# Lagrange-Labs/mapreduce-plonky2

Measured on AMD Instinct MI355X. Metric: leaf proofs/sec (whole node) + NTT GB/s vs HBM peak, 2^20-row table build, 1/2/4/8 GPU, higher is better.
Workload: dtype u64 (Goldilocks field)

## Files before the change

### __graft_entry__.py

```python
import importlib
import os
import subprocess
import sys

ROOT = os.path.dirname(os.path.abspath(__file__))
PKG = os.path.join(ROOT, "mapreduce-plonky2_amd")


def build():
    env = dict(os.environ)
    subprocess.check_call(["make", "-s", "-j8", "-C", os.path.join(PKG, "csrc")], env=env)
    subprocess.check_call(["make", "-s", "-C", os.path.join(ROOT, "oracle")], env=env)
    subprocess.check_call(["make", "-s", "-C", os.path.join(ROOT, "tests", "devfield")], env=env)
    subprocess.check_call(["make", "-s", "-C", os.path.join(ROOT, "tests", "devfield_mulc")], env=env)
    subprocess.check_call(["make", "-s", "-C", os.path.join(ROOT, "tests", "devfield_mulk")], env=env)
    sys.path.insert(0, ROOT)
    mod = importlib.import_module("mapreduce-plonky2_amd")
    assert os.path.exists(mod.LIB_PATH)
    mod.load()


def smoke():
    import numpy as np
    sys.path.insert(0, ROOT)
    sys.path.insert(0, os.path.join(ROOT, "tests"))
    mp2 = importlib.import_module("mapreduce-plonky2_amd")
    import oracle as O
    ctx = mp2.Context(0)
    log_n, w = 10, 12
    vals = O.rand_field((w, 1 << log_n), 0xC0FFEE01)
    b = mp2.PolynomialBatch.from_values(ctx, vals, 3, 4)
    coeffs = O.fft(vals, inverse=True)
    cap = O.merkle_cap(O.merkle_build(O.lde_leaves(coeffs, 3), 4), 4)
    assert np.array_equal(b.coeffs, coeffs), "iNTT mismatch vs oracle"
    assert np.array_equal(b.cap, cap), "Merkle cap mismatch vs oracle"
    b.free()
    import ctypes
    import circuits as C
    ckt = C.build(5, C.ALL_KINDS, 1)
    ofp = O.standard_params(5, (ckt.num_constants + C.NUM_ROUTED, C.NUM_WIRES, 20, 16), pow_bits=6, num_queries=4)
    fp = mp2.FriParams()
    ctypes.memmove(ctypes.byref(fp), ctypes.byref(ofp), ctypes.sizeof(fp))
    cd = O.rand_field(4, 2)
    pr = mp2.BatchedProver(ctx, fp, 1)
    pr.set_preprocessed(ctx.to_device(ckt.pre))
    pr.enable_permutation(C.NUM_ROUTED, 8)
    pr.enable_quotient()
    pr.set_gates(ckt.gates, ckt.num_selectors)
    pr.prove([ctx.to_device(ckt.wires[None]), None, None], ctx.to_device(cd), ctx.to_device(ckt.pi_hash[None]))
    caps, openings, proofs = pr.results()
    oc, oo, op, bgao = C.prove(ckt, ofp, cd)
    assert np.array_equal(caps[0], oc) and np.array_equal(openings[0], oo) and np.array_equal(proofs[0], op), "proof mismatch vs oracle"
    assert O.pcs_verify(ofp, cd, ckt.pi_hash, caps[0], openings[0], proofs[0]) == 0, "FRI verifier rejects"
    assert C.identity_check(ckt, ofp, openings[0], bgao) == 0, "PLONK identity fails"
    ver = mp2.Verifier(ctx, fp, caps[0][0], cd, ckt.gates, ckt.num_selectors, capacity=2)
    words = np.concatenate([ckt.pi_hash, caps[0][1:].ravel(), openings[0].ravel(), proofs[0]])
    bad = words.copy()
    bad[4 + 3 * fp.cap_words + 9] ^= np.uint64(1)
    st = ver.verify(np.stack([words, bad])).tolist()
    assert st[0] == 0 and st[1] != 0, f"device verifier: {st}"
    ver.free()
    pr.free()
    R = importlib.import_module("mapreduce-plonky2_amd.recursion")
    FW = importlib.import_module("mapreduce-plonky2_amd.framework")
    data = O.rand_field(4, 0xC0FFEE03)
    mc = R.map_circuit(data)
    prog = mp2.WitnessProgram(mc)
    wires, pi_hash, pis = prog.run(data[None])
    assert np.array_equal(wires[0], mc.wires), "witness program != builder"
    n = 1 << mc.log_n
    d_in, d_w, d_pr = ctx.to_device(data[None]), ctx.alloc(135 * n * 8), ctx.alloc(prog.probe.size * 8)
    prog.run_dev(ctx, d_in, 1, d_w, d_pr)
    assert np.array_equal(d_w.download((135, n)), mc.wires), "device witness replay != builder"
    assert np.array_equal(d_pr.download((prog.probe.size,))[:4], pi_hash[0])
    cp = FW.CircuitProver(ctx, mc, 1, witness_check=True, pow_bits=8, num_queries=6)
    cp.prove(ctx.to_device(wires), ctx.to_device(pi_hash))
    assert cp.pr.witness_status().tolist() == [0]
    c2, o2, p2 = cp.results()
    mfp = C.oracle_params(mc, pow_bits=8, num_queries=6)
    assert C.verify(mc, mfp, cp.circuit_digest, pi_hash[0], c2[0], o2[0], p2[0]) == 0, "oracle verifier rejects the map proof"
    assert int(pis[0][0]) == sum(int(x) for x in data if int(x) % 2 == 0) % O.P
    cp.free()
    ctx.close()
    print("smoke ok: commit_from_values(12 x 2^10) == oracle; prove(2^5 rows, 24 gates) == oracle and verifies (oracle and device verifier); "
          "map circuit (real, witness program on host and device) proves and verifies")


if __name__ == "__main__":
    build()
    if len(sys.argv) > 1 and sys.argv[1] == "smoke":
        smoke()
```

### mapreduce-plonky2_amd/csrc/fri.hip

```cpp
#include "fri.h"
#include "poseidon_wave.cuh"

namespace mp2g {

template <int V>
__device__ void ch_duplex(ChState& c) {
  for (u32 i = 0; i < c.n_in; i++) c.state[i] = c.in[i];
  c.n_in = 0;
  u64 s[12];
#pragma unroll
  for (int i = 0; i < 12; i++) s[i] = c.state[i];
  perm<V>(s);
#pragma unroll
  for (int i = 0; i < 12; i++) c.state[i] = s[i];
#pragma unroll
  for (int i = 0; i < 8; i++) c.out[i] = s[i];
  c.n_out = 8;
}
template <int V>
__global__ void ch_kernel(ChState* st, u32 B, const u64* obs, u64 obs_bstride, u32 n_obs, u64* out, u64 out_bstride, u32 n_get) {
  u32 b = blockIdx.x * blockDim.x + threadIdx.x;
  if (b >= B) return;
  ChState c = st[b];
  const u64* o = obs + b * obs_bstride;
  for (u32 i = 0; i < n_obs; i++) {
    c.n_out = 0;
    c.in[c.n_in++] = o[i];
    if (c.n_in == 8) ch_duplex<V>(c);
  }
  u64* dst = out + b * out_bstride;
  for (u32 i = 0; i < n_get; i++) {
    if (c.n_in || !c.n_out) ch_duplex<V>(c);
    dst[i] = c.out[--c.n_out];
  }
  st[b] = c;
}
__global__ void __launch_bounds__(64) ch_wave_kernel(ChState* st, u32 B, const u64* obs, u64 obs_bstride, u32 n_obs, u64* out,
                                                     u64 out_bstride, u32 n_get) {
  const u32 gid = blockIdx.x * blockDim.x + threadIdx.x;
  const u32 braw = gid >> 4, l = gid & 15;
  const bool active = braw < B;
  const u32 b = active ? braw : B - 1;
  ChState* c = st + b;
  u64 x = l < 12 ? c->state[l] : 0;
  u64 inb = l < 8 ? c->in[l] : 0, outb = l < 8 ? c->out[l] : 0;
  u32 n_in = c->n_in, n_out = c->n_out;
  const u64* o = obs + b * obs_bstride;
  auto duplex = [&]() {
    if (l < n_in) x = inb;
    n_in = 0;
    x = wp2_perm(x, (int)l);
    outb = x;
    n_out = 8;
  };
  for (u32 i = 0; i < n_obs; i++) {
    u64 e = o[i];
    n_out = 0;
    if (l == n_in) inb = e;
    if (++n_in == 8) duplex();
  }
  u64* dst = out + b * out_bstride;
  for (u32 i = 0; i < n_get; i++) {
    if (n_in || !n_out) duplex();
    --n_out;
    if (active && l == n_out) dst[i] = outb;
  }
  if (!active) return;
  if (l < 12) c->state[l] = x;
  if (l < 8) { c->in[l] = inb; c->out[l] = outb; }
  if (l == 0) { c->n_in = n_in; c->n_out = n_out; }
}
__global__ void ch_init_kernel(ChState* st, u32 B) {
  u32 b = blockIdx.x * blockDim.x + threadIdx.x;
  if (b >= B) return;
  ChState c;
  for (int i = 0; i < 12; i++) c.state[i] = 0;
  for (int i = 0; i < 8; i++) { c.in[i] = 0; c.out[i] = 0; }
  c.n_in = c.n_out = 0;
  st[b] = c;
}
hipError_t challenger_init(hipStream_t s, ChState* st, u32 B) {
  hipLaunchKernelGGL(ch_init_kernel, dim3((B + 63) / 64), dim3(64), 0, s, st, B);
  return hipGetLastError();
}
hipError_t challenger_step(hipStream_t s, int variant, ChState* st, u32 B, const u64* obs, u64 obs_bstride, u32 n_obs,
                           u64* out, u64 out_bstride, u32 n_get) {
  if (variant == MP2G_POSEIDON2)
    hipLaunchKernelGGL(ch_wave_kernel, dim3((B * 16 + 63) / 64), dim3(64), 0, s, st, B, obs, obs_bstride, n_obs, out, out_bstride, n_get);
  else
    hipLaunchKernelGGL((ch_kernel<MP2G_POSEIDON>), dim3((B + 63) / 64), dim3(64), 0, s, st, B, obs, obs_bstride, n_obs, out, out_bstride, n_get);
  return hipGetLastError();
}

#define EP_RUN 16
__global__ void __launch_bounds__(256) ext_powers_kernel(const u64* __restrict__ x, u64 x_bstride, u64 scale, u32 count,
                                                         u64* __restrict__ out, u64 out_bstride) {
  const u32 b = blockIdx.y, e0 = blockIdx.x * 256 * EP_RUN + threadIdx.x;
  if (e0 >= count) return;
  const gl2 xb = gl2_scale(gl2_make(x[b * x_bstride], x[b * x_bstride + 1]), scale);
  const gl2 step = gl2_pow(xb, 256);
  gl2 pw = gl2_pow(xb, e0);
  u64* o = out + b * out_bstride;
  for (u32 r = 0, e = e0; r < EP_RUN && e < count; r++, e += 256) {
    o[e] = pw.a;
    o[count + e] = pw.b;
    pw = gl2_mul(pw, step);
  }
}
static hipError_t ext_powers(hipStream_t s, u32 B, const u64* x, u64 x_bstride, u64 scale, u32 count, u64* out, u64 out_bstride) {
  hipLaunchKernelGGL(ext_powers_kernel, dim3((count + 256 * EP_RUN - 1) / (256 * EP_RUN), B), dim3(256), 0, s, x, x_bstride, scale, count, out,
                     out_bstride);
  return hipGetLastError();
}

#define OP_POLYS 4
__global__ void __launch_bounds__(256) openings_kernel(FriShape sh, const u64* __restrict__ zpw, u64 zpw_bstride, u64* out ) {
  const u32 b = blockIdx.y, t = threadIdx.x;
  const u32 n = 1u << sh.log_n, n_open = sh.n_polys + sh.zs_count + sh.lookup_count;
  const u32 blocks0 = (sh.n_polys + OP_POLYS - 1) / OP_POLYS;
  const bool shifted = blockIdx.x >= blocks0;
  const u32 j0 = shifted ? sh.n_polys + (blockIdx.x - blocks0) * OP_POLYS : blockIdx.x * OP_POLYS;
  const u32 nq = min(OP_POLYS, (shifted ? n_open : sh.n_polys) - j0);
  const u64* pa = zpw + b * zpw_bstride + (shifted ? 2 * (u64)n : 0);
  const u64* pb = pa + n;
  const u64* c[OP_POLYS];
#pragma unroll
  for (u32 q = 0; q < OP_POLYS; q++) {
    u32 o, p;
    const u32 j = j0 + (q < nq ? q : 0);
    if (shifted) fri_batch_poly(sh, 1, j - sh.n_polys, o, p);
    else fri_batch_poly(sh, 0, j, o, p);
    c[q] = sh.o[o].coeffs + b * sh.o[o].coeff_bstride + ((u64)p << sh.log_n);
  }
  gl_cols sa[OP_POLYS], sb[OP_POLYS];
  for (u32 i = t; i < n; i += 256) {
    const u64 za = pa[i], zb = pb[i];
#pragma unroll
    for (u32 q = 0; q < OP_POLYS; q++)
      if (q < nq) {
        const u64 v = c[q][i];
        sa[q].add(v, za);
        sb[q].add(v, zb);
      }
  }
  __shared__ u64 ra[OP_POLYS][256], rb[OP_POLYS][256];
#pragma unroll
  for (u32 q = 0; q < OP_POLYS; q++) { ra[q][t] = sa[q].value(); rb[q][t] = sb[q].value(); }
  __syncthreads();
  for (u32 s = 128; s > 0; s >>= 1) {
    if (t < s)
#pragma unroll
      for (u32 q = 0; q < OP_POLYS; q++) { ra[q][t] = gl_add(ra[q][t], ra[q][t + s]); rb[q][t] = gl_add(rb[q][t], rb[q][t + s]); }
    __syncthreads();
  }
  if (t < nq) {
    u64* d = out + ((u64)b * n_open + j0 + t) * 2;
    d[0] = ra[t][0]; d[1] = rb[t][0];
  }
}

__global__ void __launch_bounds__(256) compose_kernel(FriShape sh, const u64* __restrict__ apw, u64 apw_bstride, u32 apw_len, u64* comp) {
  const u32 n = 1u << sh.log_n;
  const u32 i = blockIdx.x * 256 + threadIdx.x, b = blockIdx.y, batch = blockIdx.z;
  if (i >= n) return;
  const u64* pa = apw + b * apw_bstride;
  const u64* pb = pa + apw_len;
  gl_cols sa, sb;
  u32 m = 0;
  const u32 zo = sh.zs_oracle, wz = sh.o[zo].w - sh.lookup_count;
  auto run = [&](u32 o, u32 first, u32 count) {
    const u64* base = sh.o[o].coeffs + b * sh.o[o].coeff_bstride + i;
    for (u32 p = first; p < first + count; p++, m++) {
      const u64 v = base[(u64)p << sh.log_n];
      sa.add(v, pa[m]);
      sb.add(v, pb[m]);
    }
  };
  if (batch == 0) {
    for (u32 o = 0; o < sh.n_oracles; o++) run(o, 0, o == zo ? wz : sh.o[o].w);
  } else {
    run(zo, 0, sh.zs_count);
  }
  if (sh.lookup_count) run(zo, wz, sh.lookup_count);
  u64* d = comp + (((u64)b * 2 + batch) * 2) * n;
  d[i] = sa.value();
  d[n + i] = sb.value();
}

__global__ void __launch_bounds__(1024) divide_kernel(u32 log_n, const u64* zeta, u64 zeta_bstride, const u64* comp, u64* quot) {
  const u32 n = 1u << log_n, batch = blockIdx.x, b = blockIdx.y, t = threadIdx.x;
  const u32 T = n < 1024 ? n : 1024, S = n / T;
  gl2 z = gl2_make(zeta[b * zeta_bstride], zeta[b * zeta_bstride + 1]);
  if (batch == 1) z = gl2_scale(z, gl_root_of_unity(log_n));
  const u64* c0 = comp + (((u64)b * 2 + batch) * 2) * n;
  const u64* c1 = c0 + n;
  u64* q0 = quot + (((u64)b * 2 + batch) * 2) * n;
  u64* q1 = q0 + n;
  __shared__ u64 la[1024], lb[1024];
  gl2 L = gl2_make(0, 0);
  if (t < T) {
    for (int k = (int)S - 1; k >= 0; k--) {
      L = gl2_mul(L, z);
      L.a = gl_add(L.a, c0[t * S + k]);
      L.b = gl_add(L.b, c1[t * S + k]);
    }
  }
  la[t] = 0; lb[t] = 0;
  __syncthreads();
  if (t < T && t >= 1) { la[t - 1] = L.a; lb[t - 1] = L.b; }
  __syncthreads();
  gl2 zp = gl2_pow(z, S);
  for (u32 d = 1; d < T; d <<= 1) {
    gl2 add = gl2_make(0, 0);
    if (t + d < T) add = gl2_mul(zp, gl2_make(la[t + d], lb[t + d]));
    __syncthreads();
    if (t < T) { la[t] = gl_add(la[t], add.a); lb[t] = gl_add(lb[t], add.b); }
    __syncthreads();
    zp = gl2_mul(zp, zp);
  }
  if (t < T) {
    gl2 s = gl2_make(la[t], lb[t]);
    for (int k = (int)S - 1; k >= 0; k--) {
      u32 i = t * S + k;
      s = gl2_mul(s, z);
      s.a = gl_add(s.a, c0[i]);
      s.b = gl_add(s.b, c1[i]);
      if (i >= 1) { q0[i - 1] = s.a; q1[i - 1] = s.b; }
    }
    if (t == T - 1) { q0[n - 1] = 0; q1[n - 1] = 0; }
  }
}
__global__ void __launch_bounds__(256) combine_kernel(u32 log_n, u32 zs_count, const u64* __restrict__ apw, u64 apw_bstride, u32 apw_len,
                                                      const u64* quot, u64* final_poly) {
  const u32 n = 1u << log_n, i = blockIdx.x * 256 + threadIdx.x, b = blockIdx.y;
  if (i >= n) return;
  const gl2 sh = gl2_make(apw[b * apw_bstride + zs_count], apw[b * apw_bstride + apw_len + zs_count]);
  const u64* q = quot + (u64)b * 4 * n;
  gl2 r = gl2_add(gl2_mul(gl2_make(q[i], q[n + i]), sh), gl2_make(q[2 * n + i], q[3 * n + i]));
  final_poly[(u64)b * 2 * n + i] = r.a;
  final_poly[(u64)b * 2 * n + n + i] = r.b;
}

template <int AB>
__global__ void __launch_bounds__(256) fold_values_kernel(u32 log_m, const u64* in, u64 in_bstride, u64* out, u64 out_bstride,
                                                            const u64* beta, u64 beta_bstride, u64 shift_inv, u64 w_m_inv, u64 arity_inv) {
  constexpr int A = 1 << AB;
  const u32 m = 1u << log_m, chunks = m >> AB;
  const u32 c = blockIdx.x * 256 + threadIdx.x, b = blockIdx.y;
  if (c >= chunks) return;
  const u64* v0 = in + b * in_bstride + ((u64)c << AB);
  const u64* v1 = v0 + m;
  gl2 x[A];
#pragma unroll
  for (int k = 0; k < A; k++) x[k] = gl2_make(v0[k], v1[k]);
  const u64 wA_inv = gl_pow(w_m_inv, m >> AB);
#pragma unroll
  for (int s = 1; s <= AB; s++) {
    const int mm = 1 << s, h = mm >> 1;
    u64 wstep = wA_inv;
    for (int e = s; e < AB; e++) wstep = gl_sqr(wstep);
    u64 w = 1;
#pragma unroll
    for (int j = 0; j < h; j++) {
#pragma unroll
      for (int k = 0; k < A; k += mm) {
        gl2 t = j == 0 ? x[k + j + h] : gl2_scale(x[k + j + h], w);
        gl2 u = x[k + j];
        x[k + j] = gl2_add(u, t);
        x[k + j + h] = gl2_sub(u, t);
      }
      w = gl_mul(w, wstep);
    }
  }
  u64 x0_inv = gl_mul(shift_inv, gl_pow(w_m_inv, bitrev32(c, log_m - AB)));
  gl2 g = gl2_scale(gl2_make(beta[b * beta_bstride], beta[b * beta_bstride + 1]), x0_inv);
  gl2 acc = x[A - 1];
#pragma unroll
  for (int j = A - 2; j >= 0; j--) acc = gl2_add(gl2_mul(acc, g), x[j]);
  acc = gl2_scale(acc, arity_inv);
  u64* o = out + b * out_bstride;
  o[c] = acc.a;
  o[chunks + c] = acc.b;
}
__global__ void __launch_bounds__(256) fold_coeffs_kernel(u32 n_out, u32 ab, const u64* in, u64 in_bstride, u32 n_in, u64* out, u64 out_bstride,
                                                            const u64* beta, u64 beta_bstride, int aos_out) {
  const u32 i = blockIdx.x * 256 + threadIdx.x, b = blockIdx.y;
  if (i >= n_out) return;
  const u32 A = 1u << ab;
  const u64* c0 = in + b * in_bstride + ((u64)i << ab);
  const u64* c1 = c0 + n_in;
  gl2 be = gl2_make(beta[b * beta_bstride], beta[b * beta_bstride + 1]);
  gl2 acc = gl2_make(0, 0);
  for (int j = (int)A - 1; j >= 0; j--) acc = gl2_add(gl2_mul(acc, be), gl2_make(c0[j], c1[j]));
  u64* o = out + b * out_bstride;
  if (aos_out) { o[2 * i] = acc.a; o[2 * i + 1] = acc.b; }
  else { o[i] = acc.a; o[n_out + i] = acc.b; }
}
__global__ void soa_to_aos_kernel(u32 n, const u64* in, u64 in_bstride, u32 n_in, u64* out, u64 out_bstride) {
  const u32 i = blockIdx.x * blockDim.x + threadIdx.x, b = blockIdx.y;
  if (i >= n) return;
  out[b * out_bstride + 2 * i] = in[b * in_bstride + i];
  out[b * out_bstride + 2 * i + 1] = in[b * in_bstride + n_in + i];
}

#define POW_THREADS 256
#define POW_STRIDE 16
#define POW_TICKET 1
template <int V>
__global__ void __launch_bounds__(POW_THREADS) pow_kernel(const ChState* st, u32 bits, unsigned long long* witness) {
  const u32 b = blockIdx.y;
  const ChState& c = st[b];
  unsigned long long* wit = witness + (u64)b * POW_STRIDE;
  __shared__ unsigned long long s_best, s_chunk;
  u64 base[12];
#pragma unroll
  for (int i = 0; i < 12; i++) base[i] = c.state[i];
  const u32 pos = c.n_in;
#pragma unroll
  for (int i = 0; i < 8; i++)
    if ((u32)i < pos) base[i] = c.in[i];
  for (;;) {
    if (threadIdx.x == 0) {
      s_chunk = atomicAdd(wit + POW_TICKET, 1ull);
      s_best = atomicMin(wit, ~0ull);
    }
    __syncthreads();
    const unsigned long long best = s_best;
    const u64 cand = (u64)s_chunk * POW_THREADS + threadIdx.x;
    __syncthreads();
    if (cand - threadIdx.x > best) break;
    u64 s[12];
#pragma unroll
    for (int i = 0; i < 12; i++) s[i] = base[i];
#pragma unroll
    for (int i = 0; i < 8; i++)
      if ((u32)i == pos) s[i] = cand;
    perm<V>(s);
    if (cand < GL_P && (bits == 0 || (s[7] >> (64 - bits)) == 0)) atomicMin(wit, (unsigned long long)cand);
  }
}
__global__ void pow_reset_kernel(u64* witness, u32 n) {
  u32 i = blockIdx.x * blockDim.x + threadIdx.x;
  if (i < n) witness[i] = (i % POW_STRIDE) ? 0 : ~(u64)0;
}

__global__ void __launch_bounds__(256) query_kernel(FriShape sh, FriLayers ly, FriProofLayout L, const u64* chal ,
                                                      u64 chal_bstride, u64* proof) {
  const u32 q = blockIdx.x, b = blockIdx.y, t = threadIdx.x;
  const u32 lg = L.lg;
  const u64 N = (u64)1 << lg;
  u64 x = chal[b * chal_bstride + q] % N;
  u64* const qs = proof + b * L.proof_words + L.q_off + q * L.q_words;
  auto siblings = [&](u64* o, const u64* lv, u32 clg, u32 n_sib, u64 x) {
    for (u32 e = t; e < n_sib * 4; e += 256) {
      u32 l = e >> 2, k = e & 3;
      u64 off = 0;
      for (u32 j = 0; j < l; j++) off += (u64)4 << (clg - j);
      o[e] = lv[off + 4 * ((x >> l) ^ 1) + k];
    }
  };
  for (u32 oi = 0; oi < sh.n_oracles; oi++) {
    const OracleRef& r = sh.o[oi];
    u64* o = qs + L.leaf_off[oi];
    const u64* vals = r.values + b * r.value_bstride;
    for (u32 p = t; p < r.w; p += 256) o[p] = vals[(u64)p * N + x];
    siblings(o + r.w, r.levels + b * r.level_bstride, lg, L.n_sib[oi], x);
  }
  u32 clg = lg;
  for (u32 li = 0; li < ly.n_layers; li++) {
    const u32 ab = ly.arity_bits[li], A = 1u << ab, p = sh.n_oracles + li;
    const u64 m = (u64)1 << clg;
    x >>= ab;
    clg -= ab;
    u64* o = qs + L.leaf_off[p];
    const u64* v = ly.values[li] + b * ly.value_bstride[li];
    for (u32 e = t; e < 2 * A; e += 256) o[e] = v[(e & 1) * m + (x << ab) + (e >> 1)];
    siblings(o + 2 * A, ly.levels[li] + b * ly.level_bstride[li], clg, L.n_sib[p], x);
  }
}
__global__ void copy_rows_kernel(const u64* src, u64 src_bstride, u64* dst, u64 dst_bstride, u32 words) {
  u32 i = blockIdx.x * blockDim.x + threadIdx.x, b = blockIdx.y;
  if (i < words) dst[b * dst_bstride + i] = src[b * src_bstride + i];
}

__global__ void bind_pi_kernel(u64* wires, u64 wires_bstride, u64 n, u32 row, const u64* pi_hash, u32 B) {
  u32 t = blockIdx.x * blockDim.x + threadIdx.x;
  if (t < 4 * B) wires[(t >> 2) * wires_bstride + (u64)(t & 3) * n + row] = pi_hash[t];
}

#define HIPCHK(x) do { hipError_t e_ = (x); if (e_ != hipSuccess) return e_; } while (0)

hipError_t fri_openings(hipStream_t s, const FriShape& sh, u32 B, const u64* zeta, u64 zeta_bstride, u64* zpw, u64* out) {
  const u32 n = 1u << sh.log_n, n_shifted = sh.zs_count + sh.lookup_count;
  HIPCHK(ext_powers(s, B, zeta, zeta_bstride, 1, n, zpw, 4 * (u64)n));
  if (n_shifted) HIPCHK(ext_powers(s, B, zeta, zeta_bstride, gl_root_of_unity(sh.log_n), n, zpw + 2 * (u64)n, 4 * (u64)n));
  const u32 blocks = (sh.n_polys + OP_POLYS - 1) / OP_POLYS + (n_shifted + OP_POLYS - 1) / OP_POLYS;
  hipLaunchKernelGGL(openings_kernel, dim3(blocks, B), dim3(256), 0, s, sh, zpw, 4 * (u64)n, out);
  return hipGetLastError();
}
hipError_t fri_final_poly(hipStream_t s, const FriShape& sh, u32 B, const u64* alpha, u64 alpha_bstride, const u64* zeta, u64 zeta_bstride,
                          u64* apw, u64* comp, u64* quot, u64* final_poly) {
  const u32 n = 1u << sh.log_n, apw_len = fri_alpha_powers_len(sh);
  HIPCHK(ext_powers(s, B, alpha, alpha_bstride, 1, apw_len, apw, 2 * (u64)apw_len));
  hipLaunchKernelGGL(compose_kernel, dim3((n + 255) / 256, B, 2), dim3(256), 0, s, sh, apw, 2 * (u64)apw_len, apw_len, comp);
  hipLaunchKernelGGL(divide_kernel, dim3(2, B), dim3(1024), 0, s, sh.log_n, zeta, zeta_bstride, comp, quot);
  hipLaunchKernelGGL(combine_kernel, dim3((n + 255) / 256, B), dim3(256), 0, s, sh.log_n, sh.zs_count + sh.lookup_count, apw, 2 * (u64)apw_len,
                     apw_len, quot, final_poly);
  return hipGetLastError();
}
hipError_t fri_fold_values(hipStream_t s, u32 B, u32 log_m, u32 ab, const u64* in, u64 in_bstride, u64* out, u64 out_bstride,
                           const u64* beta, u64 beta_bstride, u64 shift) {
  const u32 chunks = (1u << log_m) >> ab;
  const u64 shift_inv = gl_inv(shift), w_m_inv = gl_inv(gl_root_of_unity(log_m)), a_inv = gl_inv((u64)1 << ab);
  dim3 g((chunks + 255) / 256, B), bl(256);
#define FV(N) case N: hipLaunchKernelGGL((fold_values_kernel<N>), g, bl, 0, s, log_m, in, in_bstride, out, out_bstride, beta, beta_bstride, shift_inv, w_m_inv, a_inv); break;
  switch (ab) { FV(1) FV(2) FV(3) FV(4) default: return hipErrorInvalidValue; }
#undef FV
  return hipGetLastError();
}
hipError_t fri_fold_coeffs(hipStream_t s, u32 B, u32 n_in, u32 ab, const u64* in, u64 in_bstride, u64* out, u64 out_bstride,
                           const u64* beta, u64 beta_bstride, bool aos_out) {
  const u32 n_out = n_in >> ab;
  hipLaunchKernelGGL(fold_coeffs_kernel, dim3((n_out + 255) / 256, B), dim3(256), 0, s, n_out, ab, in, in_bstride, n_in, out, out_bstride, beta, beta_bstride, aos_out ? 1 : 0);
  return hipGetLastError();
}
hipError_t fri_soa_to_aos(hipStream_t s, u32 B, u32 n, const u64* in, u64 in_bstride, u32 n_in, u64* out, u64 out_bstride) {
  hipLaunchKernelGGL(soa_to_aos_kernel, dim3((n + 255) / 256, B), dim3(256), 0, s, n, in, in_bstride, n_in, out, out_bstride);
  return hipGetLastError();
}
hipError_t fri_pow(hipStream_t s, int variant, const ChState* st, u32 B, u32 bits, u64* witness) {
  hipLaunchKernelGGL(pow_reset_kernel, dim3((B * POW_STRIDE + 63) / 64), dim3(64), 0, s, witness, B * POW_STRIDE);
  const u32 lanes = 1u << 19;
  u32 blocks = lanes / POW_THREADS / (B ? B : 1);
  if (blocks < 8) blocks = 8;
  if (blocks > 1024) blocks = 1024;
  dim3 g(blocks, B), bl(POW_THREADS);
  if (variant == MP2G_POSEIDON2) hipLaunchKernelGGL((pow_kernel<MP2G_POSEIDON2>), g, bl, 0, s, st, bits, (unsigned long long*)witness);
  else hipLaunchKernelGGL((pow_kernel<MP2G_POSEIDON>), g, bl, 0, s, st, bits, (unsigned long long*)witness);
  return hipGetLastError();
}
hipError_t fri_queries(hipStream_t s, const FriShape& sh, const FriLayers& ly, const FriProofLayout& L, u32 B, u32 num_queries,
                       const u64* chal, u64 chal_bstride, u64* proof) {
  if (!num_queries) return hipSuccess;
  hipLaunchKernelGGL(query_kernel, dim3(num_queries, B), dim3(256), 0, s, sh, ly, L, chal, chal_bstride, proof);
  return hipGetLastError();
}
hipError_t bind_public_inputs(hipStream_t s, u32 B, u64* wires, u64 wires_bstride, u64 n, u32 row, const u64* pi_hash) {
  hipLaunchKernelGGL(bind_pi_kernel, dim3((4 * B + 63) / 64), dim3(64), 0, s, wires, wires_bstride, n, row, pi_hash, B);
  return hipGetLastError();
}
hipError_t copy_rows(hipStream_t s, u32 B, const u64* src, u64 src_bstride, u64* dst, u64 dst_bstride, u32 words) {
  if (!words) return hipSuccess;
  hipLaunchKernelGGL(copy_rows_kernel, dim3((words + 255) / 256, B), dim3(256), 0, s, src, src_bstride, dst, dst_bstride, words);
  return hipGetLastError();
}
}
```

### mapreduce-plonky2_amd/csrc/merkle.hip

```cpp
#include "merkle.h"
#include <atomic>
#include "poseidon_wave.cuh"

namespace mp2g {

template <int V>
__global__ void __launch_bounds__(256) leaf_hash_poly_major_kernel(const u64* __restrict__ values, u32 w, u64 stride, u64 n, u64* __restrict__ digests,
                                                                   u64 in_bstride, u64 out_bstride) {
  u64 i = (u64)blockIdx.x * blockDim.x + threadIdx.x;
  if (i >= n) return;
  values += blockIdx.y * in_bstride;
  digests += blockIdx.y * out_bstride;
  u64 s[12];
#pragma unroll
  for (int k = 0; k < 12; k++) s[k] = 0;
  if (w <= 4) {
    for (u32 p = 0; p < w; p++) s[p] = values[p * stride + i];
  } else {
    const u64* v = values + i;
    u32 p = 0;
    for (; p + 8 <= w; p += 8) {
#pragma unroll
      for (int k = 0; k < 8; k++) s[k] = v[(u64)(p + k) * stride];
      perm<V>(s);
    }
    if (p < w) {
#pragma unroll
      for (int k = 0; k < 8; k++)
        if (p + k < w) s[k] = v[(u64)(p + k) * stride];
      perm<V>(s);
    }
  }
  ulonglong2* d = reinterpret_cast<ulonglong2*>(digests + 4 * i);
  d[0] = make_ulonglong2(s[0], s[1]);
  d[1] = make_ulonglong2(s[2], s[3]);
}
template <int V>
__global__ void __launch_bounds__(256) leaf_hash_row_major_kernel(const u64* __restrict__ leaves, u32 len, u64 n, u64* __restrict__ digests) {
  u64 i = (u64)blockIdx.x * blockDim.x + threadIdx.x;
  if (i >= n) return;
  const u64* v = leaves + i * len;
  u64 s[12];
#pragma unroll
  for (int k = 0; k < 12; k++) s[k] = 0;
  if (len <= 4) {
    for (u32 p = 0; p < len; p++) s[p] = v[p];
  } else {
    u32 p = 0;
    for (; p + 8 <= len; p += 8) {
#pragma unroll
      for (int k = 0; k < 8; k++) s[k] = v[p + k];
      perm<V>(s);
    }
    if (p < len) {
#pragma unroll
      for (int k = 0; k < 8; k++)
        if (p + k < len) s[k] = v[p + k];
      perm<V>(s);
    }
  }
#pragma unroll
  for (int k = 0; k < 4; k++) digests[4 * i + k] = s[k];
}
template <int V>
__global__ void __launch_bounds__(256) leaf_hash_ext_soa_kernel(const u64* __restrict__ c0, const u64* __restrict__ c1, u32 arity_bits, u64 n, u64* __restrict__ digests,
                                                                u64 in_bstride, u64 out_bstride) {
  u64 i = (u64)blockIdx.x * blockDim.x + threadIdx.x;
  if (i >= n) return;
  c0 += blockIdx.y * in_bstride;
  c1 += blockIdx.y * in_bstride;
  digests += blockIdx.y * out_bstride;
  u32 arity = 1u << arity_bits;
  const u64* a = c0 + (i << arity_bits);
  const u64* b = c1 + (i << arity_bits);
  u64 s[12];
#pragma unroll
  for (int k = 0; k < 12; k++) s[k] = 0;
  if (arity == 1) {
    s[0] = a[0]; s[1] = b[0];
  } else if (arity == 2) {
    s[0] = a[0]; s[1] = b[0]; s[2] = a[1]; s[3] = b[1];
  } else {
    for (u32 p = 0; p < arity; p += 4) {
#pragma unroll
      for (int k = 0; k < 4; k++) { s[2 * k] = a[p + k]; s[2 * k + 1] = b[p + k]; }
      perm<V>(s);
    }
  }
#pragma unroll
  for (int k = 0; k < 4; k++) digests[4 * i + k] = s[k];
}
template <int V>
__global__ void __launch_bounds__(256) merkle_level_kernel(const u64* __restrict__ in, u64* __restrict__ out, u64 n_out, u64 bstride) {
  u64 i = (u64)blockIdx.x * blockDim.x + threadIdx.x;
  if (i >= n_out) return;
  in += blockIdx.y * bstride;
  out += blockIdx.y * bstride;
  const ulonglong2* src = reinterpret_cast<const ulonglong2*>(in + 8 * i);
  ulonglong2 q0 = src[0], q1 = src[1], q2 = src[2], q3 = src[3];
  u64 s[12] = {q0.x, q0.y, q1.x, q1.y, q2.x, q2.y, q3.x, q3.y, 0, 0, 0, 0};
  perm<V>(s);
  ulonglong2* d = reinterpret_cast<ulonglong2*>(out + 4 * i);
  d[0] = make_ulonglong2(s[0], s[1]);
  d[1] = make_ulonglong2(s[2], s[3]);
}
__global__ void __launch_bounds__(256) merkle_level_wave_kernel(const u64* __restrict__ in, u64* __restrict__ out, u64 n_out, u64 bstride) {
  const u64 gid = (u64)blockIdx.x * blockDim.x + threadIdx.x;
  const u64 iraw = gid >> 4;
  const int l = (int)(gid & 15);
  const bool active = iraw < n_out;
  const u64 i = active ? iraw : n_out - 1;
  in += blockIdx.y * bstride;
  out += blockIdx.y * bstride;
  u64 x = l < 8 ? in[8 * i + l] : 0;
  x = wp2_perm(x, l);
  if (active && l < 4) out[4 * i + l] = x;
}
template <int V>
__global__ void __launch_bounds__(256) hash_no_pad_batch_kernel(const u64* __restrict__ in, u32 in_len, u64 count, u32 out_len, u64* __restrict__ out) {
  u64 i = (u64)blockIdx.x * blockDim.x + threadIdx.x;
  if (i >= count) return;
  const u64* v = in + i * in_len;
  u64 s[12];
#pragma unroll
  for (int k = 0; k < 12; k++) s[k] = 0;
  for (u32 p = 0; p < in_len; p += 8) {
#pragma unroll
    for (int k = 0; k < 8; k++)
      if (p + k < in_len) s[k] = v[p + k];
    perm<V>(s);
  }
  u64* o = out + i * out_len;
  u32 done = 0;
  for (;;) {
#pragma unroll
    for (int k = 0; k < 8; k++) {
      if (done < out_len) o[done] = s[k];
      done++;
    }
    if (done >= out_len) break;
    perm<V>(s);
  }
}
__global__ void merkle_open_kernel(const u64* __restrict__ levels, u32 log_leaves, u32 cap_h, const u32* __restrict__ idx, u32 n_idx, u64* __restrict__ sib) {
  u32 depth = log_leaves - cap_h;
  u32 t = blockIdx.x * blockDim.x + threadIdx.x;
  if (t >= n_idx * depth * 4) return;
  u32 k = t & 3, l = (t >> 2) % depth, q = (t >> 2) / depth;
  u64 off = 0;
  for (u32 j = 0; j < l; j++) off += (u64)4 << (log_leaves - j);
  u32 node = (idx[q] >> l) ^ 1;
  sib[t] = levels[off + 4 * (u64)node + k];
}
__global__ void gather_rows_kernel(const u64* __restrict__ values, u32 w, u64 stride, const u32* __restrict__ idx, u32 n_idx, u64* __restrict__ out) {
  u32 t = blockIdx.x * blockDim.x + threadIdx.x;
  if (t >= n_idx * w) return;
  u32 p = t % w, q = t / w;
  out[t] = values[(u64)p * stride + idx[q]];
}
__global__ void __launch_bounds__(256) transpose_kernel(const u64* __restrict__ values, u32 w, u64 stride, u64 n, u64* __restrict__ out,
                                                        u64 in_bstride, u64 out_bstride) {
  __shared__ u64 tile[64][65];
  values += blockIdx.z * in_bstride;
  out += blockIdx.z * out_bstride;
  u64 i0 = (u64)blockIdx.x * 64;
  u32 p0 = blockIdx.y * 64;
  for (int e = threadIdx.x; e < 64 * 64; e += 256) {
    int pi = e >> 6, ii = e & 63;
    if (p0 + pi < w && i0 + ii < n) tile[pi][ii] = values[(u64)(p0 + pi) * stride + i0 + ii];
  }
  __syncthreads();
  for (int e = threadIdx.x; e < 64 * 64; e += 256) {
    int ii = e >> 6, pi = e & 63;
    if (p0 + pi < w && i0 + ii < n) out[(i0 + ii) * w + p0 + pi] = tile[pi][ii];
  }
}

#define LAUNCH_V(kernel, grid, block, st, ...)                                              \
  do {                                                                                      \
    if (variant == MP2G_POSEIDON2) hipLaunchKernelGGL((kernel<MP2G_POSEIDON2>), grid, block, 0, st, __VA_ARGS__); \
    else if (variant == MP2G_POSEIDON) hipLaunchKernelGGL((kernel<MP2G_POSEIDON>), grid, block, 0, st, __VA_ARGS__); \
    else return hipErrorInvalidValue;                                                       \
  } while (0)
static inline dim3 grid1(u64 n, u32 block, u32 batch = 1) { return dim3((u32)((n + block - 1) / block), batch); }

static std::atomic<unsigned long long> g_leaf_perms{0};
unsigned long long leaf_permutations_queued() { return g_leaf_perms.load(std::memory_order_relaxed); }

hipError_t leaf_hash_poly_major(hipStream_t st, int variant, const u64* values, u32 w, u64 stride, u64 n, u64* digests,
                                u32 batch, u64 in_bstride, u64 out_bstride) {
  if (!n || !batch) return hipSuccess;
  if (w > 4) g_leaf_perms.fetch_add((unsigned long long)n * batch * ((w + 7) / 8), std::memory_order_relaxed);
  LAUNCH_V(leaf_hash_poly_major_kernel, grid1(n, 256, batch), dim3(256), st, values, w, stride, n, digests, in_bstride, out_bstride);
  return hipGetLastError();
}
hipError_t leaf_hash_row_major(hipStream_t st, int variant, const u64* leaves, u32 len, u64 n, u64* digests) {
  if (!n) return hipSuccess;
  LAUNCH_V(leaf_hash_row_major_kernel, grid1(n, 256), dim3(256), st, leaves, len, n, digests);
  return hipGetLastError();
}
hipError_t leaf_hash_ext_soa(hipStream_t st, int variant, const u64* c0, const u64* c1, u32 arity_bits, u64 n, u64* digests,
                             u32 batch, u64 in_bstride, u64 out_bstride) {
  if (!n || !batch) return hipSuccess;
  LAUNCH_V(leaf_hash_ext_soa_kernel, grid1(n, 256, batch), dim3(256), st, c0, c1, arity_bits, n, digests, in_bstride, out_bstride);
  return hipGetLastError();
}
hipError_t merkle_reduce(hipStream_t st, int variant, u64* levels, u32 log_leaves, u32 cap_h, u32 batch, u64 bstride) {
  u64* cur = levels;
  if (!batch) return hipSuccess;
  for (u32 lv = log_leaves; lv > cap_h; lv--) {
    u64 n_in = (u64)1 << lv;
    u64* nxt = cur + 4 * n_in;
    if (variant == MP2G_POSEIDON2 && (n_in / 2) * (u64)batch <= 16384) {
      hipLaunchKernelGGL(merkle_level_wave_kernel, grid1(n_in / 2 * 16, 256, batch), dim3(256), 0, st, cur, nxt, n_in / 2, bstride);
    } else
      LAUNCH_V(merkle_level_kernel, grid1(n_in / 2, 256, batch), dim3(256), st, cur, nxt, n_in / 2, bstride);
    cur = nxt;
  }
  return hipGetLastError();
}
hipError_t hash_no_pad_batch(hipStream_t st, int variant, const u64* in, u32 in_len, u64 count, u32 out_len, u64* out) {
  if (!count) return hipSuccess;
  LAUNCH_V(hash_no_pad_batch_kernel, grid1(count, 256), dim3(256), st, in, in_len, count, out_len, out);
  return hipGetLastError();
}
hipError_t merkle_open(hipStream_t st, const u64* levels, u32 log_leaves, u32 cap_h, const u32* idx, u32 n_idx, u64* siblings) {
  u32 total = n_idx * (log_leaves - cap_h) * 4;
  if (!total) return hipSuccess;
  hipLaunchKernelGGL(merkle_open_kernel, grid1(total, 256), dim3(256), 0, st, levels, log_leaves, cap_h, idx, n_idx, siblings);
  return hipGetLastError();
}
hipError_t gather_rows(hipStream_t st, const u64* values, u32 w, u64 stride, const u32* idx, u32 n_idx, u64* out) {
  u32 total = n_idx * w;
  if (!total) return hipSuccess;
  hipLaunchKernelGGL(gather_rows_kernel, grid1(total, 256), dim3(256), 0, st, values, w, stride, idx, n_idx, out);
  return hipGetLastError();
}
hipError_t transpose_to_leaves(hipStream_t st, const u64* values, u32 w, u64 stride, u64 n, u64* out, u32 batch, u64 in_bstride,
                               u64 out_bstride) {
  if (!n || !w || !batch) return hipSuccess;
  hipLaunchKernelGGL(transpose_kernel, dim3((u32)((n + 63) / 64), (w + 63) / 64, batch), dim3(256), 0, st, values, w, stride, n, out,
                     in_bstride, out_bstride);
  return hipGetLastError();
}
}
```

### mapreduce-plonky2_amd/csrc/poseidon.cuh

```cuda
#pragma once
#include "gl.cuh"
#include "perm_constants.h"

#pragma push_macro("MP2G_DEVCONST")
#undef MP2G_DEVCONST
#undef MP2G_PERM_CONSTANTS_H
#define MP2G_DEVCONST static constexpr
namespace p2_cx {
#include "perm_constants.h"
constexpr u64 diag_shl32(int i) { return (u64)(((unsigned __int128)POSEIDON2_DIAG_M1[i] << 32) % GL_P); }
constexpr unsigned diag_narrow(int i = 0) {
  return i == 12 ? 0u : (GL_MULC_NARROW(POSEIDON2_DIAG_M1[i], diag_shl32(i)) ? 1u << i : 0u) | diag_narrow(i + 1);
}
}
#pragma pop_macro("MP2G_DEVCONST")
MP2G_DEVCONST uint64_t POSEIDON2_DIAG_M1_SHL32[12] = {
  p2_cx::diag_shl32(0), p2_cx::diag_shl32(1), p2_cx::diag_shl32(2), p2_cx::diag_shl32(3), p2_cx::diag_shl32(4), p2_cx::diag_shl32(5),
  p2_cx::diag_shl32(6), p2_cx::diag_shl32(7), p2_cx::diag_shl32(8), p2_cx::diag_shl32(9), p2_cx::diag_shl32(10), p2_cx::diag_shl32(11),
};
constexpr unsigned POSEIDON2_DIAG_NARROW = p2_cx::diag_narrow();
static_assert(POSEIDON2_DIAG_NARROW == 0xcfeu, "limbs 0, 8 and 9 take gl_mulc_addw's carry (profiles/p2_diag measured this split)");

#define MP2G_POSEIDON2 0
#define MP2G_POSEIDON 1

#define c_p2_ext POSEIDON2_RC_EXT
#define c_p2_int POSEIDON2_RC_INT
#define c_p2_diag POSEIDON2_DIAG_M1
#define c_p2_diag_shl32 POSEIDON2_DIAG_M1_SHL32
#define c_p_rc POSEIDON_RC

GLHD u64 p2_sbox(u64 x, u64 rc) {
  u64 t = gl_addw(x, rc);
  u64 t2 = gl_mulw(t, t), t4 = gl_mulw(t2, t2), t3 = gl_mulw(t, t2);
  return gl_mulw(t3, t4);
}
GLHD void p2_m4_plain(u64& a, u64& b, u64& c, u64& d) {
  u64 t0 = a + b, t1 = c + d;
  u64 t2 = (b << 1) + t1, t3 = (d << 1) + t0;
  u64 t4 = (t1 << 2) + t3, t5 = (t0 << 2) + t2;
  a = t3 + t5; b = t5; c = t2 + t4; d = t4;
}
GLHD void p2_external_half(u64 v[12]) {
  p2_m4_plain(v[0], v[1], v[2], v[3]);
  p2_m4_plain(v[4], v[5], v[6], v[7]);
  p2_m4_plain(v[8], v[9], v[10], v[11]);
#pragma unroll
  for (int i = 0; i < 4; i++) {
    u64 sum = v[i] + v[4 + i] + v[8 + i];
    v[i] += sum; v[4 + i] += sum; v[8 + i] += sum;
  }
}
template <bool RC>
GLHD void p2_external_rc(u64 s[12], const u64* rc) {
  u64 lo[12], hi[12];
#pragma unroll
  for (int i = 0; i < 12; i++) { lo[i] = (u32)s[i]; hi[i] = s[i] >> 32; }
  p2_external_half(lo);
  p2_external_half(hi);
#if defined(__HIP_DEVICE_COMPILE__)
#pragma unroll
  for (int i = 0; i < 12; i++) {
    u64 L = lo[i], H = hi[i];
    if (RC) { L += (u64)(u32)rc[i]; H += rc[i] >> 32; }
    H += L >> 32;
    s[i] = gl_reduce96w(gl_mk((u32)L, (u32)H), H >> 32);
  }
#else
#pragma unroll
  for (int i = 0; i < 12; i++) {
    u32 c0, c1, top = (u32)(hi[i] >> 32);
    u32 l0 = (u32)lo[i];
    u32 l1 = __builtin_addc((u32)(lo[i] >> 32), (u32)hi[i], 0u, &c0);
    top += c0;
    if (RC) {
      const u64 k = rc[i];
      l0 = __builtin_addc(l0, (u32)k, 0u, &c0);
      l1 = __builtin_addc(l1, (u32)(k >> 32), c0, &c1);
      top += c1;
    }
    s[i] = gl_reduce96w(gl_mk(l0, l1), top);
  }
#endif
}
GLHD void p2_external(u64 s[12]) { p2_external_rc<false>(s, nullptr); }
GLHD u64 p2_sbox0(u64 t) {
  u64 t2 = gl_mulw_k(t, t), t4 = gl_mulw_k(t2, t2), t3 = gl_mulw_k(t, t2);
  return gl_mulw_k(t3, t4);
}
GLHD u64 p2_diag_mul_addw(int i, u64 a, u64 c) {
  if ((POSEIDON2_DIAG_NARROW >> i) & 1) return gl_mulc_addw<true>(a, c_p2_diag[i], c_p2_diag_shl32[i], c);
  return gl_mulc_addw<false>(a, c_p2_diag[i], c_p2_diag_shl32[i], c);
}
GLD u64 p2_limb_sum(const u64 s[12]) {
#if defined(__HIP_DEVICE_COMPILE__)
  u64 w = s[0], ha, hb;
#pragma unroll
  for (int i = 1; i < 12; i++) w += s[i];
#define P2_MAD1_(r, x, z) asm volatile("v_mad_u64_u32 %0, vcc, %1, 1, %2" : "=v"(r) : "v"((u32)((x) >> 32)), "v"(z) : "vcc")
  asm volatile("v_mad_u64_u32 %0, vcc, %1, 1, 0" : "=v"(ha) : "v"((u32)(s[0] >> 32)) : "vcc");
  asm volatile("v_mad_u64_u32 %0, vcc, %1, 1, 0" : "=v"(hb) : "v"((u32)(s[1] >> 32)) : "vcc");
#pragma unroll
  for (int i = 2; i < 12; i += 2) {
    P2_MAD1_(ha, s[i], ha);
    P2_MAD1_(hb, s[i + 1], hb);
  }
  const u64 h = ha + hb;
  const u32 c = (u32)(w >> 32) - (u32)h;
  u64 t;
  asm volatile("v_mad_u64_u32 %0, vcc, %1, 1, %2" : "=v"(t) : "v"(c), "v"(h) : "vcc");
#undef P2_MAD1_
  return gl_reduce96w(w, t >> 32);
#else
  unsigned __int128 x = 0;
  for (int i = 0; i < 12; i++) x += s[i];
  return gl_reduce96w((u64)x, (u64)(x >> 64));
#endif
}
GLHD void p2_internal(u64 s[12]) {
#if defined(__HIP_DEVICE_COMPILE__)
  const u64 sum = p2_limb_sum(s);
#pragma unroll
  for (int i = 0; i < 12; i++) {
    s[i] = p2_diag_mul_addw(i, s[i], sum);
    __builtin_amdgcn_sched_barrier(0);
  }
#else
  u64 acc = s[0];
  u64 top = 0;
#pragma unroll
  for (int i = 1; i < 12; i++) {
    bool c = __builtin_add_overflow(acc, s[i], &acc);
    top += c ? 1 : 0;
  }
#pragma unroll
  for (int i = 0; i < 12; i++) {
    u64 lo, hi;
    gl_mul_wide(s[i], c_p2_diag[i], lo, hi);
    bool c = __builtin_add_overflow(lo, acc, &lo);
    s[i] = gl_reduce128w(lo, hi + top + (c ? 1 : 0));
  }
#endif
}
GLHD void poseidon2_perm(u64 s[12]) {
  p2_external_rc<true>(s, c_p2_ext);
#pragma unroll 1
  for (int r = 0; r < 4; r++) {
#pragma unroll
    for (int i = 0; i < 12; i++) s[i] = p2_sbox0(s[i]);
    if (r < 3) p2_external_rc<true>(s, c_p2_ext + 12 * (r + 1)); else p2_external(s);
  }
#pragma unroll 11
  for (int r = 0; r < 22; r++) {
    s[0] = p2_sbox0(gl_addw(s[0], c_p2_int[r]));
    p2_internal(s);
  }
#pragma unroll
  for (int i = 0; i < 12; i++) s[i] = gl_addw(s[i], c_p2_ext[48 + i]);
#pragma unroll 1
  for (int r = 4; r < 8; r++) {
#pragma unroll
    for (int i = 0; i < 12; i++) s[i] = p2_sbox0(s[i]);
    if (r < 7) p2_external_rc<true>(s, c_p2_ext + 12 * (r + 1)); else p2_external(s);
  }
#pragma unroll
  for (int i = 0; i < 12; i++) s[i] = gl_canon(s[i]);
}

template <bool RC>
GLHD void poseidon_mds_rc(u64 s[12], const u64* rc) {
  const u32 circ[12] = {17, 15, 41, 16, 2, 28, 13, 13, 39, 18, 34, 20};
  u64 lo[12], hi[12];
#pragma unroll
  for (int i = 0; i < 12; i++) { lo[i] = (u32)s[i]; hi[i] = s[i] >> 32; }
  u64 out[12];
#pragma unroll
  for (int r = 0; r < 12; r++) {
    u64 al = 0, ah = 0;
#pragma unroll
    for (int i = 0; i < 12; i++) {
      al += lo[(i + r) % 12] * circ[i];
      ah += hi[(i + r) % 12] * circ[i];
    }
    if (r == 0) { al += lo[0] * 8; ah += hi[0] * 8; }
    u32 c0, c1, top = (u32)(ah >> 32);
    u32 l0 = (u32)al;
    u32 l1 = __builtin_addc((u32)(al >> 32), (u32)ah, 0u, &c0);
    top += c0;
    if (RC) {
      const u64 k = rc[r];
      l0 = __builtin_addc(l0, (u32)k, 0u, &c0);
      l1 = __builtin_addc(l1, (u32)(k >> 32), c0, &c1);
      top += c1;
    }
    out[r] = gl_reduce96w(gl_mk(l0, l1), top);
  }
#pragma unroll
  for (int i = 0; i < 12; i++) s[i] = out[i];
}
GLHD void poseidon_mds(u64 s[12]) { poseidon_mds_rc<false>(s, nullptr); }
GLHD void poseidon_perm(u64 s[12]) {
#pragma unroll
  for (int i = 0; i < 12; i++) s[i] = gl_addw(s[i], c_p_rc[i]);
#pragma unroll 1
  for (int r = 0; r < 30; r++) {
    if (r < 4 || r >= 26) {
#pragma unroll
      for (int i = 0; i < 12; i++) s[i] = p2_sbox0(s[i]);
    } else {
      s[0] = p2_sbox0(s[0]);
    }
    if (r < 29) poseidon_mds_rc<true>(s, c_p_rc + 12 * (r + 1)); else poseidon_mds(s);
  }
#pragma unroll
  for (int i = 0; i < 12; i++) s[i] = gl_canon(s[i]);
}
template <int VARIANT>
GLHD void perm(u64 s[12]) {
  if (VARIANT == MP2G_POSEIDON2) poseidon2_perm(s); else poseidon_perm(s);
}
template <int VARIANT>
GLD void two_to_one(const u64 l[4], const u64 r[4], u64 out[4]) {
  u64 s[12];
#pragma unroll
  for (int i = 0; i < 4; i++) { s[i] = l[i]; s[4 + i] = r[i]; s[8 + i] = 0; }
  perm<VARIANT>(s);
#pragma unroll
  for (int i = 0; i < 4; i++) out[i] = s[i];
}
```

Before: 1058.

## Skip unused output lanes of final Poseidon2 layer and precompute PoW first layer

Splits the Poseidon2 permutation into the first external layer, a body and a masked final external layer. Sponge absorbs, digests and two-to-one compressions now reduce and canonicalize only the state lanes that are read next (capacity lanes for full absorbs, the first four for digests). The PoW grind precomputes the first external MDS layer of the fixed base state once in shared memory and adds the candidate's linear contribution per lane, so each candidate skips that layer. This adds masking logic and per-position weight tables whose correctness depends on how the sponge states are used afterwards.

Result: no change. 1059 (median of 3 runs) (+0.1%).

```diff
diff --git a/__graft_entry__.py b/__graft_entry__.py
--- a/__graft_entry__.py
+++ b/__graft_entry__.py
@@ -14,6 +14,7 @@
     subprocess.check_call(["make", "-s", "-C", os.path.join(ROOT, "tests", "devfield")], env=env)
     subprocess.check_call(["make", "-s", "-C", os.path.join(ROOT, "tests", "devfield_mulc")], env=env)
     subprocess.check_call(["make", "-s", "-C", os.path.join(ROOT, "tests", "devfield_mulk")], env=env)
+    subprocess.check_call(["make", "-s", "-C", os.path.join(ROOT, "tests", "devp2")], env=env)
     sys.path.insert(0, ROOT)
     mod = importlib.import_module("mapreduce-plonky2_amd")
     assert os.path.exists(mod.LIB_PATH)
diff --git a/mapreduce-plonky2_amd/csrc/fri.hip b/mapreduce-plonky2_amd/csrc/fri.hip
--- a/mapreduce-plonky2_amd/csrc/fri.hip
+++ b/mapreduce-plonky2_amd/csrc/fri.hip
@@ -306,12 +306,22 @@
 #define POW_THREADS 256
 #define POW_STRIDE 16
 #define POW_TICKET 1
+GLD u64 pow_add_word(u32 x, u64 z) {
+#if defined(__HIP_DEVICE_COMPILE__)
+  u64 r;
+  asm("v_mad_u64_u32 %0, vcc, %1, 1, %2" : "=v"(r) : "v"(x), "v"(z) : "vcc");
+  return r;
+#else
+  return x + z;
+#endif
+}
 template <int V>
 __global__ void __launch_bounds__(POW_THREADS) pow_kernel(const ChState* st, u32 bits, unsigned long long* witness) {
   const u32 b = blockIdx.y;
   const ChState& c = st[b];
   unsigned long long* wit = witness + (u64)b * POW_STRIDE;
   __shared__ unsigned long long s_best, s_chunk;
+  __shared__ u64 s_base[12];
   u64 base[12];
 #pragma unroll
   for (int i = 0; i < 12; i++) base[i] = c.state[i];
@@ -319,6 +329,20 @@
 #pragma unroll
   for (int i = 0; i < 8; i++)
     if ((u32)i < pos) base[i] = c.in[i];
+  u32 wt[12];
+  if (V == MP2G_POSEIDON2) {
+    const u32 m4_cols = pos % 4 == 0 ? 0x01010405u : pos % 4 == 1 ? 0x01030607u : pos % 4 == 2 ? 0x04050101u : 0x06070103u;
+#pragma unroll
+    for (int i = 0; i < 12; i++) {
+      wt[i] = pos < 8 ? ((m4_cols >> (8 * (i % 4))) & 0xffu) << ((u32)(i / 4) == pos / 4 ? 1 : 0) : 0u;
+      if ((u32)i == pos) base[i] = 0;
+    }
+    p2_external_rc<true>(base, c_p2_ext);
+    if (threadIdx.x == 0) {
+#pragma unroll
+      for (int i = 0; i < 12; i++) s_base[i] = base[i];
+    }
+  }
   for (;;) {
     if (threadIdx.x == 0) {
       s_chunk = atomicAdd(wit + POW_TICKET, 1ull);
@@ -330,12 +354,20 @@
     __syncthreads();
     if (cand - threadIdx.x > best) break;
     u64 s[12];
-#pragma unroll
-    for (int i = 0; i < 12; i++) s[i] = base[i];
-#pragma unroll
-    for (int i = 0; i < 8; i++)
-      if ((u32)i == pos) s[i] = cand;
-    perm<V>(s);
+    if (V == MP2G_POSEIDON2) {
+#pragma unroll
+      for (int i = 0; i < 12; i++)
+        s[i] = p2_external_finish(pow_add_word((u32)s_base[i], (u64)(u32)cand * wt[i]), pow_add_word((u32)(s_base[i] >> 32), (cand >> 32) * wt[i]));
+      poseidon2_body(s);
+      p2_external_last<0x080u, true>(s);
+    } else {
+#pragma unroll
+      for (int i = 0; i < 12; i++) s[i] = base[i];
+#pragma unroll
+      for (int i = 0; i < 8; i++)
+        if ((u32)i == pos) s[i] = cand;
+      perm<V>(s);
+    }
     if (cand < GL_P && (bits == 0 || (s[7] >> (64 - bits)) == 0)) atomicMin(wit, (unsigned long long)cand);
   }
 }
diff --git a/mapreduce-plonky2_amd/csrc/merkle.hip b/mapreduce-plonky2_amd/csrc/merkle.hip
--- a/mapreduce-plonky2_amd/csrc/merkle.hip
+++ b/mapreduce-plonky2_amd/csrc/merkle.hip
@@ -22,13 +22,13 @@
     for (; p + 8 <= w; p += 8) {
 #pragma unroll
       for (int k = 0; k < 8; k++) s[k] = v[(u64)(p + k) * stride];
-      perm<V>(s);
+      sponge_perm<V>(s, p + 16 <= w ? SPONGE_ABSORB_FULL : p + 8 == w ? SPONGE_DIGEST : SPONGE_ABSORB_PARTIAL);
     }
     if (p < w) {
 #pragma unroll
       for (int k = 0; k < 8; k++)
         if (p + k < w) s[k] = v[(u64)(p + k) * stride];
-      perm<V>(s);
+      sponge_perm<V>(s, SPONGE_DIGEST);
     }
   }
   ulonglong2* d = reinterpret_cast<ulonglong2*>(digests + 4 * i);
@@ -50,13 +50,13 @@
     for (; p + 8 <= len; p += 8) {
 #pragma unroll
       for (int k = 0; k < 8; k++) s[k] = v[p + k];
-      perm<V>(s);
+      sponge_perm<V>(s, p + 16 <= len ? SPONGE_ABSORB_FULL : p + 8 == len ? SPONGE_DIGEST : SPONGE_ABSORB_PARTIAL);
     }
     if (p < len) {
 #pragma unroll
       for (int k = 0; k < 8; k++)
         if (p + k < len) s[k] = v[p + k];
-      perm<V>(s);
+      sponge_perm<V>(s, SPONGE_DIGEST);
     }
   }
 #pragma unroll
@@ -84,7 +84,7 @@
     for (u32 p = 0; p < arity; p += 4) {
 #pragma unroll
       for (int k = 0; k < 4; k++) { s[2 * k] = a[p + k]; s[2 * k + 1] = b[p + k]; }
-      perm<V>(s);
+      sponge_perm<V>(s, p + 4 < arity ? SPONGE_ABSORB_FULL : SPONGE_DIGEST);
     }
   }
 #pragma unroll
@@ -99,7 +99,7 @@
   const ulonglong2* src = reinterpret_cast<const ulonglong2*>(in + 8 * i);
   ulonglong2 q0 = src[0], q1 = src[1], q2 = src[2], q3 = src[3];
   u64 s[12] = {q0.x, q0.y, q1.x, q1.y, q2.x, q2.y, q3.x, q3.y, 0, 0, 0, 0};
-  perm<V>(s);
+  compress_perm<V>(s);
   ulonglong2* d = reinterpret_cast<ulonglong2*>(out + 4 * i);
   d[0] = make_ulonglong2(s[0], s[1]);
   d[1] = make_ulonglong2(s[2], s[3]);
@@ -128,7 +128,7 @@
 #pragma unroll
     for (int k = 0; k < 8; k++)
       if (p + k < in_len) s[k] = v[p + k];
-    perm<V>(s);
+    sponge_perm<V>(s, p + 16 <= in_len ? SPONGE_ABSORB_FULL : SPONGE_SQUEEZE);
   }
   u64* o = out + i * out_len;
   u32 done = 0;
diff --git a/mapreduce-plonky2_amd/csrc/poseidon.cuh b/mapreduce-plonky2_amd/csrc/poseidon.cuh
--- a/mapreduce-plonky2_amd/csrc/poseidon.cuh
+++ b/mapreduce-plonky2_amd/csrc/poseidon.cuh
@@ -84,6 +84,30 @@
 #endif
 }
 GLHD void p2_external(u64 s[12]) { p2_external_rc<false>(s, nullptr); }
+GLHD u64 p2_external_finish(u64 L, u64 H) {
+#if defined(__HIP_DEVICE_COMPILE__)
+  H += L >> 32;
+  return gl_reduce96w(gl_mk((u32)L, (u32)H), H >> 32);
+#else
+  u32 c0, top = (u32)(H >> 32);
+  u32 l1 = __builtin_addc((u32)(L >> 32), (u32)H, 0u, &c0);
+  return gl_reduce96w(gl_mk((u32)L, l1), top + c0);
+#endif
+}
+template <unsigned MASK, bool CANON>
+GLHD void p2_external_last(u64 s[12]) {
+  u64 lo[12], hi[12];
+#pragma unroll
+  for (int i = 0; i < 12; i++) { lo[i] = (u32)s[i]; hi[i] = s[i] >> 32; }
+  p2_external_half(lo);
+  p2_external_half(hi);
+#pragma unroll
+  for (int i = 0; i < 12; i++) {
+    if (!((MASK >> i) & 1)) continue;
+    const u64 x = p2_external_finish(lo[i], hi[i]);
+    s[i] = CANON ? gl_canon(x) : x;
+  }
+}
 GLHD u64 p2_sbox0(u64 t) {
   u64 t2 = gl_mulw_k(t, t), t4 = gl_mulw_k(t2, t2), t3 = gl_mulw_k(t, t2);
   return gl_mulw_k(t3, t4);
@@ -142,8 +166,7 @@
   }
 #endif
 }
-GLHD void poseidon2_perm(u64 s[12]) {
-  p2_external_rc<true>(s, c_p2_ext);
+GLHD void poseidon2_body(u64 s[12]) {
 #pragma unroll 1
   for (int r = 0; r < 4; r++) {
 #pragma unroll
@@ -158,14 +181,20 @@
 #pragma unroll
   for (int i = 0; i < 12; i++) s[i] = gl_addw(s[i], c_p2_ext[48 + i]);
 #pragma unroll 1
-  for (int r = 4; r < 8; r++) {
+  for (int r = 4;; r++) {
 #pragma unroll
     for (int i = 0; i < 12; i++) s[i] = p2_sbox0(s[i]);
-    if (r < 7) p2_external_rc<true>(s, c_p2_ext + 12 * (r + 1)); else p2_external(s);
-  }
-#pragma unroll
-  for (int i = 0; i < 12; i++) s[i] = gl_canon(s[i]);
-}
+    if (r == 7) break;
+    p2_external_rc<true>(s, c_p2_ext + 12 * (r + 1));
+  }
+}
+template <unsigned MASK, bool CANON>
+GLHD void poseidon2_perm_limbs(u64 s[12]) {
+  p2_external_rc<true>(s, c_p2_ext);
+  poseidon2_body(s);
+  p2_external_last<MASK, CANON>(s);
+}
+GLHD void poseidon2_perm(u64 s[12]) { poseidon2_perm_limbs<0xfffu, true>(s); }
 
 template <bool RC>
 GLHD void poseidon_mds_rc(u64 s[12], const u64* rc) {
@@ -219,12 +248,32 @@
 GLHD void perm(u64 s[12]) {
   if (VARIANT == MP2G_POSEIDON2) poseidon2_perm(s); else poseidon_perm(s);
 }
+enum SpongeNext {
+  SPONGE_ABSORB_FULL,
+  SPONGE_ABSORB_PARTIAL,
+  SPONGE_DIGEST,
+  SPONGE_SQUEEZE,
+};
+template <int VARIANT>
+GLHD void sponge_perm(u64 s[12], SpongeNext next) {
+  if (VARIANT != MP2G_POSEIDON2) { poseidon_perm(s); return; }
+  p2_external_rc<true>(s, c_p2_ext);
+  poseidon2_body(s);
+  if (next == SPONGE_ABSORB_FULL) p2_external_last<0xf00u, false>(s);
+  else if (next == SPONGE_DIGEST) p2_external_last<0x00fu, true>(s);
+  else if (next == SPONGE_ABSORB_PARTIAL) p2_external_last<0xfffu, false>(s);
+  else p2_external_last<0xfffu, true>(s);
+}
+template <int VARIANT>
+GLHD void compress_perm(u64 s[12]) {
+  if (VARIANT == MP2G_POSEIDON2) poseidon2_perm_limbs<0x00fu, true>(s); else poseidon_perm(s);
+}
 template <int VARIANT>
 GLD void two_to_one(const u64 l[4], const u64 r[4], u64 out[4]) {
   u64 s[12];
 #pragma unroll
   for (int i = 0; i < 4; i++) { s[i] = l[i]; s[4 + i] = r[i]; s[8 + i] = 0; }
-  perm<VARIANT>(s);
+  compress_perm<VARIANT>(s);
 #pragma unroll
   for (int i = 0; i < 4; i++) out[i] = s[i];
 }
```
